# fergusfinn/qmps

Hardware: AMD Instinct MI355X
Metric: two-site energy evals/sec at D=4, batch=65536 (higher is better)
Workload: dtype f64

## Files before the change

### qmps_amd/csrc/qmps_direct.hip

```cpp
#include <hip/hip_runtime.h>
#include <stdint.h>

#include "qmps_hip.h"
#include "qmps_kernels.h"
#include "qmps_device.h"
#include "qmps_circuit.h"
#include "qmps_direct_core.h"
#include "qmps_direct_d8.h"

namespace qmps {

namespace {

struct QuadOps {
  using V = double;
  using P = bool;
  int q;
  const double2* row;
  double* gj;
  __device__ __forceinline__ P q_eq(int i) const { return q == i; }
  __device__ __forceinline__ P q_gt(int i) const { return q > i; }
  template <int L>
  static __device__ __forceinline__ V bcast(V v) { return quad_bcast<L>(v); }
  template <int L, int K>
  __device__ __forceinline__ void row_bcast(const V (&r)[16], V (&out)[16]) const {
#ifdef QMPS_GJ_LDS
    constexpr int K0 = K & ~1;
    __builtin_amdgcn_wave_barrier();
    if (q == L) {
#pragma unroll
      for (int j = K0; j < 16; j += 2) *(double2*)&gj[j] = make_double2(r[j], r[j + 1]);
    }
    __builtin_amdgcn_wave_barrier();
#pragma unroll
    for (int j = K0; j < 16; j += 2) {
      const double2 t = *(const double2*)&gj[j];
      if (j >= K) out[j] = t.x;
      out[j + 1] = t.y;
    }
#else
#pragma unroll
    for (int j = K; j < 16; ++j) out[j] = quad_bcast<L>(r[j]);
#endif
  }
  static __device__ __forceinline__ V qsum(V v) { return quad_sum(v); }
  static __device__ __forceinline__ V qmax(V v) {
    v = fmax(v, quad_perm<0xB1>(v));
    return fmax(v, quad_perm<0x4E>(v));
  }
  static __device__ __forceinline__ V vabs(V v) { return fabs(v); }
  static __device__ __forceinline__ V vmax(V a, V b) { return fmax(a, b); }
  static __device__ __forceinline__ V sel(P p, V a, V b) { return p ? a : b; }
  static __device__ __forceinline__ V splat(double x) { return x; }
  static __device__ __forceinline__ V fma(V a, V b, V c) { return dfma(a, b, c); }
  static __device__ __forceinline__ V rcp(V t) { return fast_rcp(t); }
  static __device__ __forceinline__ P lt(V a, V b) { return a < b; }
  static __device__ __forceinline__ P gt0(V a) { return a > 0.0; }
  static __device__ __forceinline__ P p_and(P a, P b) { return a && b; }
  static __device__ __forceinline__ P p_not(P a) { return !a; }
  static __device__ __forceinline__ bool any(P a) { return __any(a) != 0; }
  __device__ __forceinline__ void own(int s, int j, V& re, V& im) const {
    const double2 v = row[(4 * s + q) * 4 + j];
    re = v.x;
    im = v.y;
  }
  __device__ __forceinline__ void uni(int s, int i, int j, V& re, V& im) const {
    const double2 v = row[(4 * s + i) * 4 + j];
    re = v.x;
    im = v.y;
  }
};

typedef const __attribute__((address_space(4))) double* const_f64_ptr;
__device__ __forceinline__ const_f64_ptr h_term(const void* h, int t) { return (const_f64_ptr)(uintptr_t)h + 32 * t; }

typedef double v4f64 __attribute__((ext_vector_type(4)));
constexpr int kSqLD = 17;
constexpr int kSqDoubles = 16 * kSqLD + 16;

__device__ __forceinline__ void squaring_fallback(const unsigned char* tiles, int pad, double* img, int lane, bool todo,
                                                  int max_iter, double tol2, double (&x)[4], double& steps, bool& left) {
  constexpr int D = 4, LD = kSqLD;
  constexpr double RS2 = 0.70710678118654752, S2 = 1.4142135623730951;
  const int g = lane >> 4, c = lane & 15, j = c >> 2, jp = c & 3, q = lane & 3;
  double* strip = img + 16 * LD;
  const double cpx = j == jp ? 1.0 : (j < jp ? RS2 : 0.0), cpy = j > jp ? -RS2 : 0.0;
  const double cqx = j < jp ? RS2 : 0.0, cqy = j > jp ? RS2 : 0.0;
  const bool diag = j == jp;
  unsigned long long mask = __ballot(todo);
  while (mask != 0) {
    const int e = (__ffsll((long long)mask) - 1) >> 2;
    mask &= ~(0xFull << (4 * e));
    const double2* sA = (const double2*)(tiles + e * pad);
    v4f64 R;
    {
      double pr[2], pi[2], qr[2], qi[2];
#pragma unroll
      for (int s = 0; s < 2; ++s) {
        const double2 a = sA[(s * D + g) * D + jp], b = sA[(s * D + g) * D + j];
        pr[s] = dfma(cpx, a.x, cpy * a.y);
// ... 39 lines not shown
      ++m;
      image(acc);
      z = 0.25 * ((img[c * LD + 0] + img[c * LD + 5]) + (img[c * LD + 10] + img[c * LD + 15]));
      const double inv = fast_rcp(row16_sum(diag ? z : 0.0));
      z *= inv;
      R = acc * inv;
#pragma unroll
      for (int kk = 0; kk < 4; ++kk) af[kk] *= inv;
      const double d = z - prev;
      const double d2 = row16_sum(d * d);
      prev = z;
      st = (double)(1 << m);
      active = !(d2 < tol2);
    }
    __builtin_amdgcn_wave_barrier();
    if (lane < 16) strip[lane] = diag ? z : RS2 * z;
    __builtin_amdgcn_wave_barrier();
    if ((lane >> 2) == e) {
      if (m > 0) {
#pragma unroll
        for (int l = 0; l < 4; ++l) x[l] = strip[4 * q + l];
      }
      steps = 1.0 + st;
      left = active;
    }
  }
}

}

#ifndef QMPS_DIRECT_MINWAVES
#define QMPS_DIRECT_MINWAVES 2
#endif
template <int ANS, bool WARM>
__global__ __launch_bounds__(64, QMPS_DIRECT_MINWAVES) void energy_direct_d4_kernel(LaneArgs p) {
  using Core = DirectD4<QuadOps>;
  constexpr int ROW = 512, PAD = ROW + 16, ITEMS = 16;
  __shared__ __attribute__((aligned(16))) unsigned char lds[ITEMS * PAD];
  __shared__ double sq_img[kSqDoubles];
#ifdef QMPS_GJ_LDS
  __shared__ __attribute__((aligned(16))) double gjbuf[ITEMS * 18];
#endif
  const int lane = threadIdx.x, e = lane >> 2, q = lane & 3;
  const int64_t first = (int64_t)blockIdx.x * ITEMS;
  const int64_t b = first + e;
  const bool valid = b < p.B;
  if constexpr (ANS >= 0) {
    Reg<3> reg;
#pragma unroll
    for (int xx = 0; xx < 8; ++xx) {
      reg.re[xx] = (valid && xx == q) ? 1.0 : 0.0;
      reg.im[xx] = 0.0;
    }
    const int nsh = p.ans_nsh;
    const int64_t row = valid ? b : 0;
    const int64_t ridx = nsh > 0 ? row / nsh : row;
    const int shift_k = nsh > 0 ? (int)(row - ridx * nsh) : 0;
    const int isel = nsh > 0 ? *p.ans_i : -1;
    const double* pp = p.ans_params + ridx * p.ans_P;
    constexpr int per = ANS == QMPS_ANSATZ_SHALLOW_CNOT3 ? 3 : 2, trip = ANS == QMPS_ANSATZ_SHALLOW_CNOT3 ? 3 : 4;
    const int P = p.ans_P;
    for (int l = 0; l + per <= P; l += trip) {
      const int mine = l + q;
      double ang = 0.0;
      if (q < trip && mine < P) {
        ang = pp[mine];
        if (mine == isel) ang += roto_shift_value(nsh, shift_k);
      }
      const double scale = ansatz_angle_scale<ANS>(ANS == QMPS_ANSATZ_SHALLOW_CNOT3 ? q : (q & 1));
      double sn, cs;
      sincos(scale * ang, &sn, &cs);
      {
        const double c0[3] = {quad_bcast<0>(cs), quad_bcast<1>(cs), quad_bcast<2>(cs)};
        const double s0[3] = {quad_bcast<0>(sn), quad_bcast<1>(sn), quad_bcast<2>(sn)};
        ansatz_layer_cs<3, ANS>(reg, c0, s0);
      }
      if (trip == 4 && l + 2 + per <= P) {
        const double c1[2] = {quad_bcast<2>(cs), quad_bcast<3>(cs)};
        const double s1[2] = {quad_bcast<2>(sn), quad_bcast<3>(sn)};
        ansatz_layer_cs<3, ANS>(reg, c1, s1);
      }
    }
    double2* tile = (double2*)(lds + e * PAD);
#pragma unroll
    for (int xx = 0; xx < 8; ++xx) tile[((xx & 1) * 4 + (xx >> 1)) * 4 + q] = make_double2(reg.re[xx], reg.im[xx]);
  } else {
    const unsigned char* slab = (const unsigned char*)p.A + first * ROW;
    const int64_t slab_bytes = (p.B - first < ITEMS ? p.B - first : ITEMS) * (int64_t)ROW;
    double2 v[ITEMS * ROW / 1024];
#pragma unroll
    for (int c = 0; c < ITEMS * ROW / 1024; ++c) {
      const int off = c * 1024 + lane * 16;
      v[c] = make_double2(0.0, 0.0);
      if (off < slab_bytes) v[c] = *(const double2*)(slab + off);
    }
#pragma unroll
    for (int c = 0; c < ITEMS * ROW / 1024; ++c) {
      const int off = c * 1024 + lane * 16;
      *(double2*)(lds + (off / ROW) * PAD + (off % ROW)) = v[c];
    }
  }
  __syncthreads();
#ifdef QMPS_GJ_LDS
  const QuadOps o{q, (const double2*)(lds + e * PAD), gjbuf + e * 18};
#else
  const QuadOps o{q, (const double2*)(lds + e * PAD), nullptr};
#endif
  const double tol2 = p.tol * p.tol;

  double x[4], us[16];
  double steps = 1.0;
  int status = QMPS_ST_OK;
  bool have = false;
  if constexpr (WARM) {
    const double2* rin = (const double2*)p.r_in + (valid ? b : 0) * 16;
#pragma unroll
    for (int l = 0; l < 4; ++l) {
      const double2 rw = rin[q * 4 + l], cl = rin[l * 4 + q];
      x[l] = q <= l ? rw.x : cl.y;
    }
    Core::normalise(o, x);
    Core::gather(x, us);
    double y[4];
    const double d2 = Core::power_step(o, x, us, y);
    have = valid && d2 < tol2;
#pragma unroll
    for (int l = 0; l < 4; ++l) x[l] = have ? y[l] : x[l];
    __builtin_amdgcn_sched_barrier(0);
  }
  if (!WARM || __any(valid && !have)) {
    double Rc[4][16], xs[4], y[4];
    Core::build(o, Rc);
    __builtin_amdgcn_sched_barrier(0);
    double pivmax;
    Core::solve(o, Rc, xs, pivmax);
    __builtin_amdgcn_sched_barrier(0);
    Core::normalise(o, xs);
    Core::gather(xs, us);
    const double d2 = Core::power_step(o, xs, us, y);
    __builtin_amdgcn_sched_barrier(0);
    const bool accepted = d2 < tol2 && pivmax < Core::kMaxInversePivot;
    if (!have) {
#pragma unroll
      for (int l = 0; l < 4; ++l) x[l] = xs[l];
      if (WARM) steps = 2.0;
    }
    const bool todo = valid && !have && !accepted;
    if (__any(todo)) {
      bool left = false;
      squaring_fallback(lds, PAD, sq_img, lane, todo, p.max_iter - 1, tol2, x, steps, left);
      if (__any(todo && left)) {
        double yb[4];
        Core::gather(x, us);
        const double d2b = Core::power_step(o, x, us, yb);
        const bool fin = todo && left && d2b < tol2 && steps + 1.0 <= (double)p.max_iter;
#pragma unroll
        for (int l = 0; l < 4; ++l) x[l] = fin ? yb[l] : x[l];
        if (fin) {
          left = false;
          steps += 1.0;
        }
      }
      if (todo) {
        status = left ? QMPS_ST_NOT_CONVERGED : QMPS_ST_OK;
        if (WARM) steps += 1.0;
      }
    }
    if (WARM || __any(todo)) Core::gather(x, us);
  } else {
    Core::gather(x, us);
  }
  __builtin_amdgcn_sched_barrier(0);

  double pre[4][4], pim[4][4];
  const bool pd = Core::density(o, us, p.rho_need, pre, pim);
  if (status == QMPS_ST_OK && !pd) status = QMPS_ST_NOT_PD;
  if (p.acc_zero != nullptr && blockIdx.x == 0) acc_clear(p.acc_zero, p.n_terms, lane, 64);
  for (int t = 0; t < p.n_terms; ++t) {
    const double en = quad_sum(Core::energy(h_term(p.h, t), p.rho_need, pre, pim));
    if (valid && q == 0) p.E[b * p.n_terms + t] = en;
    if (p.partial != nullptr || p.acc != nullptr) {
      const double s = wave_sum((valid && q == 0) ? en : 0.0);
      if (lane == 0) {
        if (p.partial != nullptr) p.partial[(int64_t)t * gridDim.x + blockIdx.x] = s;
        if (p.acc != nullptr) acc_arrive(p.acc, p.acc_shards, t, blockIdx.x, s, p.acc_bound, p.acc_scale);
      }
    }
  }
  if (p.rho_out != nullptr) {
    double fre[4][4], fim[4][4];
#pragma unroll
    for (int t = 0; t < 4; ++t)
#pragma unroll
      for (int s = t; s < 4; ++s) {
        fre[t][s] = quad_sum(pre[t][s]);
        fim[t][s] = t == s ? 0.0 : quad_sum(pim[t][s]);
      }
    if (valid && q == 0) {
      double2* o2 = (double2*)p.rho_out + b * 16;
#pragma unroll
      for (int t = 0; t < 4; ++t)
#pragma unroll
        for (int s = 0; s < 4; ++s)
          o2[t * 4 + s] = t <= s ? make_double2(fre[t][s], fim[t][s]) : make_double2(fre[s][t], -fim[s][t]);
    }
  }
  if (!valid) return;
  if (q == 0) {
    p.iters[b] = (int32_t)steps;
    p.status[b] = status;
  }
  if (p.r_out != nullptr) {
    double2* o2 = (double2*)p.r_out + b * 16 + q * 4;
#pragma unroll
    for (int l = 0; l < 4; ++l) {
      const double f = q == 0 ? us[4 * l] : (q == 1 ? us[4 * l + 1] : (q == 2 ? us[4 * l + 2] : us[4 * l + 3]));
      const double re = q <= l ? x[l] : f;
      const double im = q == l ? 0.0 : (q < l ? f : -x[l]);
      o2[l] = make_double2(re, im);
    }
  }
// ... 349 lines not shown
```

### qmps_amd/csrc/qmps_direct_core.h

```cpp
#pragma once

#include <stdint.h>

#include <utility>

namespace qmps {

constexpr uint32_t kRhoNeedAll = 0xFFFFFFFFu;
inline uint32_t rho_need_mask(const double* h, int n_terms) {
  uint32_t need = 0;
  for (int n = 0; n < n_terms; ++n)
    for (int s = 0; s < 4; ++s)
      for (int t = 0; t < 4; ++t) {
        const int lo = t < s ? t : s, hi = t < s ? s : t;
        const double re = h[32 * n + 2 * (4 * s + t)], im = h[32 * n + 2 * (4 * s + t) + 1];
        if (!(re == 0.0)) need |= 1u << (4 * lo + hi);
        if (lo != hi && !(im == 0.0)) need |= 1u << (16 + 4 * lo + hi);
      }
  return need;
}

#if defined(__HIPCC__)
#define QMPS_CORE_FN __device__ inline __attribute__((always_inline))
#define QMPS_SCHED_FENCE() __builtin_amdgcn_sched_barrier(0)
#else
#define QMPS_CORE_FN inline __attribute__((always_inline))
#define QMPS_SCHED_FENCE() ((void)0)
#endif
#if defined(__HIP_DEVICE_COMPILE__)
#define QMPS_COMPUTED_HERE(v) asm volatile("" : "+v"(v))
#else
#define QMPS_COMPUTED_HERE(v) ((void)0)
#endif

template <int... I, class F>
QMPS_CORE_FN void static_for_impl(std::integer_sequence<int, I...>, F&& f) {
  (f(std::integral_constant<int, I>{}), ...);
}
template <int N, class F>
QMPS_CORE_FN void static_for(F&& f) {
  static_for_impl(std::make_integer_sequence<int, N>{}, static_cast<F&&>(f));
}

template <class O>
struct DirectD4 {
  using V = typename O::V;
  using P = typename O::P;

  static QMPS_CORE_FN V own_diag(const O& o, const V (&x)[4]) {
    return O::sel(o.q_eq(0), x[0], O::sel(o.q_eq(1), x[1], O::sel(o.q_eq(2), x[2], x[3])));
  }

  static QMPS_CORE_FN void build(const O& o, V (&Rc)[4][16]) {
    V ar[2][4], ai[2][4];
#pragma unroll
    for (int s = 0; s < 2; ++s)
#pragma unroll
      for (int j = 0; j < 4; ++j) o.own(s, j, ar[s][j], ai[s][j]);
#pragma unroll
    for (int ip = 0; ip < 4; ++ip) {
      const P rot = o.q_gt(ip);
      V tr[2][4], ti[2][4], br[2][4], bi[2][4];
#pragma unroll
      for (int s = 0; s < 2; ++s)
#pragma unroll
        for (int j = 0; j < 4; ++j) {
          tr[s][j] = ip == 3 ? ar[s][j] : O::sel(rot, -ai[s][j], ar[s][j]);
          ti[s][j] = ip == 3 ? ai[s][j] : O::sel(rot, ar[s][j], ai[s][j]);
          o.uni(s, ip, j, br[s][j], bi[s][j]);
        }
#pragma unroll
      for (int j = 0; j < 4; ++j) {
        V v = tr[0][j] * br[0][j];
        v = O::fma(ti[0][j], bi[0][j], v);
        v = O::fma(tr[1][j], br[1][j], v);
        v = O::fma(ti[1][j], bi[1][j], v);
        Rc[ip][5 * j] = v;
      }
#pragma unroll
      for (int lo = 0; lo < 4; ++lo)
// ... 5 lines not shown
            if (s > 0) {
              re = O::fma(tr[s][lo], br[s][hi], re);
              im = O::fma(tr[s][lo], bi[s][hi], im);
            }
            re = O::fma(ti[s][lo], bi[s][hi], re);
            re = O::fma(tr[s][hi], br[s][lo], re);
            re = O::fma(ti[s][hi], bi[s][lo], re);
            im = O::fma(-ti[s][lo], br[s][hi], im);
            im = O::fma(ti[s][hi], br[s][lo], im);
            im = O::fma(-tr[s][hi], bi[s][lo], im);
          }
          Rc[ip][4 * lo + hi] = re;
          Rc[ip][4 * hi + lo] = im;
        }
    }
  }

  static QMPS_CORE_FN void solve(const O& o, V (&M)[4][16], V (&x)[4], V& pivmax) {
    V y[4], dinv[4];
    const V one = O::splat(1.0), zero = O::splat(0.0);
    V w[4];
#pragma unroll
    for (int l = 0; l < 4; ++l) w[l] = O::sel(o.q_eq(l), one, zero);
#pragma unroll
    for (int r = 0; r < 4; ++r) {
#pragma unroll
      for (int l = 0; l < 4; ++l) M[r][4 * l + r] = M[r][4 * l + r] - w[l];
      dinv[r] = zero;
    }
#pragma unroll
    for (int j = 0; j < 4; ++j) M[3][5 * j] = M[3][5 * j] + w[3];
    static_for<16>([&](auto K) {
      constexpr int k = decltype(K)::value, pl = k >> 2, pr = k & 3;
      V prow[16];
      o.template row_bcast<pl, k>(M[pr], prow);
      const V pinv = O::rcp(prow[k]);
      const P mine = o.q_eq(pl);
      dinv[pr] = O::sel(mine, pinv, dinv[pr]);
#pragma unroll
      for (int r = 0; r < 4; ++r) {
        V f = M[r][k] * pinv;
        if (r == pr) f = O::sel(mine, zero, f);
#pragma unroll
        for (int j = k + 1; j < 16; ++j) M[r][j] = O::fma(-f, prow[j], M[r][j]);
        if (k == 15) y[r] = -f;
      }
    });
    y[3] = O::sel(o.q_eq(3), one, y[3]);
#pragma unroll
    for (int r = 0; r < 4; ++r) x[r] = y[r] * dinv[r];
    pivmax = O::qmax(O::vmax(O::vmax(O::vabs(dinv[0]), O::vabs(dinv[1])), O::vmax(O::vabs(dinv[2]), O::vabs(dinv[3]))));
  }

  static constexpr double kMaxInversePivot = 1e10;

  static QMPS_CORE_FN void gather(const V (&x)[4], V (&xs)[16]) {
    static_for<4>([&](auto L) {
      constexpr int l = decltype(L)::value;
#pragma unroll
      for (int r = 0; r < 4; ++r) xs[4 * l + r] = O::template bcast<l>(x[r]);
    });
  }

  static QMPS_CORE_FN V normalise(const O& o, V (&x)[4]) {
    const V tr = O::qsum(own_diag(o, x));
    const V inv = O::rcp(tr);
#pragma unroll
    for (int r = 0; r < 4; ++r) x[r] = x[r] * inv;
    return inv;
  }

  static QMPS_CORE_FN V dist2(const O& o, const V (&x)[4], const V (&y)[4]) {
    V d = O::splat(0.0);
#pragma unroll
    for (int r = 0; r < 4; ++r) {
      const V dd = y[r] - x[r];
      const V wt = O::sel(o.q_eq(r), O::splat(1.0), O::splat(2.0));
      d = O::fma(wt * dd, dd, d);
    }
    return O::qsum(d);
  }

  static QMPS_CORE_FN V power_step(const O& o, const V (&x)[4], const V (&us)[16], V (&y)[4]) {
    V ar[2][4], ai[2][4], xr[2][4], xi[2][4];
#pragma unroll
    for (int s = 0; s < 2; ++s)
#pragma unroll
      for (int j = 0; j < 4; ++j) o.own(s, j, ar[s][j], ai[s][j]);
#pragma unroll
    for (int s = 0; s < 2; ++s)
#pragma unroll
      for (int l = 0; l < 4; ++l) {
        V cr = O::splat(0.0), ci = O::splat(0.0);
#pragma unroll
        for (int k = 0; k < 4; ++k) {
          const V rr = us[k <= l ? 4 * k + l : 4 * l + k];
          cr = O::fma(ar[s][k], rr, cr);
          ci = O::fma(ai[s][k], rr, ci);
          if (k != l) {
            const V ri = k < l ? us[4 * l + k] : -us[4 * k + l];
            cr = O::fma(-ai[s][k], ri, cr);
            ci = O::fma(ar[s][k], ri, ci);
          }
        }
        xr[s][l] = cr;
        xi[s][l] = ci;
      }
#pragma unroll
    for (int l = 0; l < 4; ++l) {
      V cr = O::splat(0.0), ci = O::splat(0.0);
#pragma unroll
      for (int s = 0; s < 2; ++s)
#pragma unroll
        for (int k = 0; k < 4; ++k) {
          V br, bi;
          o.uni(s, l, k, br, bi);
          cr = O::fma(xr[s][k], br, cr);
          cr = O::fma(xi[s][k], bi, cr);
          ci = O::fma(xi[s][k], br, ci);
          ci = O::fma(-xr[s][k], bi, ci);
        }
      y[l] = l == 3 ? cr : O::sel(o.q_gt(l), -ci, cr);
    }
    normalise(o, y);
    return dist2(o, x, y);
  }

  static QMPS_CORE_FN void square(V (&Rc)[4][16]) {
    V out[4][16];
    static_for<16>([&](auto C) {
      constexpr int c = decltype(C)::value, cl = c >> 2, cr = c & 3;
      V rowc[16];
#pragma unroll
      for (int j = 0; j < 16; ++j) rowc[j] = O::template bcast<cl>(Rc[cr][j]);
#pragma unroll
      for (int r = 0; r < 4; ++r)
#pragma unroll
        for (int j = 0; j < 16; ++j) out[r][j] = c == 0 ? Rc[r][c] * rowc[j] : O::fma(Rc[r][c], rowc[j], out[r][j]);
      QMPS_SCHED_FENCE();
    });
#pragma unroll
    for (int r = 0; r < 4; ++r)
#pragma unroll
      for (int j = 0; j < 16; ++j) Rc[r][j] = out[r][j];
  }

  static QMPS_CORE_FN P squaring(const O& o, V (&Rc)[4][16], P active, int max_iter, double tol2, V (&x)[4], V& steps) {
    V prev[4];
#pragma unroll
    for (int r = 0; r < 4; ++r) prev[r] = O::sel(o.q_eq(r), O::splat(0.25), O::splat(0.0));
    int m = 0;
    while (O::any(active) && m < 29 && (2 << m) <= max_iter) {
      square(Rc);
      ++m;
      V z[4];
#pragma unroll
      for (int r = 0; r < 4; ++r) z[r] = O::splat(0.25) * ((Rc[r][0] + Rc[r][5]) + (Rc[r][10] + Rc[r][15]));
      const V inv = normalise(o, z);
#pragma unroll
      for (int r = 0; r < 4; ++r)
#pragma unroll
        for (int j = 0; j < 16; ++j) Rc[r][j] = Rc[r][j] * inv;
      const P conv = O::lt(dist2(o, prev, z), O::splat(tol2));
#pragma unroll
      for (int r = 0; r < 4; ++r) {
        x[r] = O::sel(active, z[r], x[r]);
        prev[r] = z[r];
      }
      steps = O::sel(active, O::splat((double)(1 << m)), steps);
      active = O::p_and(active, O::p_not(conv));
    }
    return active;
  }

  static QMPS_CORE_FN void b_rows(const O& o, V (&bre)[4][4], V (&bim)[4][4]) {
    V ar[2][4], ai[2][4];
#pragma unroll
    for (int s = 0; s < 2; ++s)
#pragma unroll
      for (int j = 0; j < 4; ++j) o.own(s, j, ar[s][j], ai[s][j]);
#pragma unroll
    for (int t2 = 0; t2 < 2; ++t2)
#pragma unroll
      for (int j = 0; j < 4; ++j) {
        V ur[4], ui[4];
#pragma unroll
        for (int k = 0; k < 4; ++k) o.uni(t2, j, k, ur[k], ui[k]);
#pragma unroll
        for (int t1 = 0; t1 < 2; ++t1)
#pragma unroll
          for (int k = 0; k < 4; ++k) {
            V cr, ci;
            if (j == 0) {
              cr = ar[t1][0] * ur[k];
              ci = ar[t1][0] * ui[k];
            } else {
              cr = O::fma(ar[t1][j], ur[k], bre[2 * t1 + t2][k]);
              ci = O::fma(ar[t1][j], ui[k], bim[2 * t1 + t2][k]);
            }
            bre[2 * t1 + t2][k] = O::fma(-ai[t1][j], ui[k], cr);
            bim[2 * t1 + t2][k] = O::fma(ai[t1][j], ur[k], ci);
          }
      }
  }

  static QMPS_CORE_FN V energy_lean(const V (&bre)[4][4], const V (&bim)[4][4], const V (&us)[16], const double* h) {
    V e = O::splat(0.0);
#pragma unroll
    for (int sg = 0; sg < 4; ++sg) {
      V cr[4], ci[4];
#pragma unroll
      for (int l = 0; l < 4; ++l) {
        cr[l] = O::splat(0.0);
        ci[l] = O::splat(0.0);
      }
#pragma unroll
      for (int tau = 0; tau < 4; ++tau) {
        const V hr = O::splat(h[2 * (4 * sg + tau)]), hi = O::splat(h[2 * (4 * sg + tau) + 1]);
#pragma unroll
        for (int l = 0; l < 4; ++l) {
          cr[l] = O::fma(hr, bre[tau][l], cr[l]);
          cr[l] = O::fma(-hi, bim[tau][l], cr[l]);
          ci[l] = O::fma(hr, bim[tau][l], ci[l]);
          ci[l] = O::fma(hi, bre[tau][l], ci[l]);
        }
      }
#pragma unroll
      for (int l = 0; l < 4; ++l) {
        V zr = O::splat(0.0), zi = O::splat(0.0);
#pragma unroll
        for (int k = 0; k < 4; ++k) {
          const V rr = us[k <= l ? 4 * k + l : 4 * l + k];
          zr = O::fma(cr[k], rr, zr);
          zi = O::fma(ci[k], rr, zi);
          if (k != l) {
            const V ri = k < l ? us[4 * l + k] : -us[4 * k + l];
            zr = O::fma(-ci[k], ri, zr);
            zi = O::fma(cr[k], ri, zi);
          }
        }
        e = O::fma(zr, bre[sg][l], e);
        e = O::fma(zi, bim[sg][l], e);
      }
    }
    return e;
  }

  static QMPS_CORE_FN P density(const O& o, const V (&us)[16], V (&pre)[4][4], V (&pim)[4][4]) {
    return density(o, us, kRhoNeedAll, pre, pim);
  }
  static QMPS_CORE_FN P density(const O& o, const V (&us)[16], uint32_t need, V (&pre)[4][4], V (&pim)[4][4]) {
    V rre[4][4], rim[4][4];
#pragma unroll
    for (int k = 0; k < 4; ++k)
#pragma unroll
      for (int l = k; l < 4; ++l) {
        rre[k][l] = us[4 * k + l];
        rim[k][l] = k == l ? O::splat(0.0) : us[4 * l + k];
      }
    P pd = O::gt0(rre[0][0]);
    V lre[4][4], lim[4][4], d[4];
    {
#pragma unroll
      for (int j = 0; j < 4; ++j) {
        V dj = rre[j][j];
#pragma unroll
        for (int k = 0; k < j; ++k) dj = O::fma(-(lre[j][k] * lre[j][k] + lim[j][k] * lim[j][k]), d[k], dj);
        d[j] = dj;
        pd = O::p_and(pd, O::gt0(dj));
        const V inv = O::rcp(O::sel(O::gt0(dj), dj, O::splat(1.0)));
#pragma unroll
        for (int i = j + 1; i < 4; ++i) {
          V cr = rre[j][i], ci = -rim[j][i];
#pragma unroll
          for (int k = 0; k < j; ++k) {
            const V pr = lre[i][k] * lre[j][k] + lim[i][k] * lim[j][k];
            const V pi = lim[i][k] * lre[j][k] - lre[i][k] * lim[j][k];
            cr = O::fma(-pr, d[k], cr);
            ci = O::fma(-pi, d[k], ci);
          }
          lre[i][j] = cr * inv;
          lim[i][j] = ci * inv;
        }
      }
    }
    V bre[4][4], bim[4][4];
    b_rows(o, bre, bim);
#pragma unroll
    for (int tau = 0; tau < 4; ++tau)
#pragma unroll
      for (int k = 0; k < 4; ++k) {
        V cr = bre[tau][k], ci = bim[tau][k];
#pragma unroll
        for (int i = k + 1; i < 4; ++i) {
          cr = O::fma(bre[tau][i], lre[i][k], cr);
          cr = O::fma(-bim[tau][i], lim[i][k], cr);
          ci = O::fma(bre[tau][i], lim[i][k], ci);
          ci = O::fma(bim[tau][i], lre[i][k], ci);
        }
        bre[tau][k] = cr;
        bim[tau][k] = ci;
      }
    computed_here(bre, bim);
#pragma unroll
    for (int tau = 0; tau < 4; ++tau) {
      V gre[4], gim[4];
#pragma unroll
      for (int k = 0; k < 4; ++k) {
        gre[k] = bre[tau][k] * d[k];
        gim[k] = bim[tau][k] * d[k];
      }
      rho_row(tau, need, gre, gim, bre, bim, pre, pim);
    }
    QMPS_SCHED_FENCE();
    if (O::any(O::p_not(pd))) {
      b_rows(o, bre, bim);
      computed_here(bre, bim);
#pragma unroll
      for (int tau = 0; tau < 4; ++tau) {
        V yre[4], yim[4];
#pragma unroll
        for (int l = 0; l < 4; ++l) {
          V cr = O::splat(0.0), ci = O::splat(0.0);
#pragma unroll
          for (int k = 0; k < 4; ++k) {
            const V rr = k <= l ? rre[k][l] : rre[l][k];
            cr = O::fma(bre[tau][k], rr, cr);
            ci = O::fma(bim[tau][k], rr, ci);
            if (k != l) {
              const V ri = k < l ? rim[k][l] : -rim[l][k];
              cr = O::fma(-bim[tau][k], ri, cr);
              ci = O::fma(bre[tau][k], ri, ci);
            }
          }
          yre[l] = cr;
          yim[l] = ci;
          QMPS_COMPUTED_HERE(yre[l]);
          QMPS_COMPUTED_HERE(yim[l]);
        }
        V qre[4][4], qim[4][4];
        rho_row(tau, need, yre, yim, bre, bim, qre, qim);
#pragma unroll
        for (int sg = tau; sg < 4; ++sg) {
          pre[tau][sg] = O::sel(pd, pre[tau][sg], qre[tau][sg]);
          pim[tau][sg] = O::sel(pd, pim[tau][sg], qim[tau][sg]);
        }
// ... 19 lines not shown
  }
  static QMPS_CORE_FN void rho_row(int tau, uint32_t need, const V (&yre)[4], const V (&yim)[4], const V (&bre)[4][4],
                                   const V (&bim)[4][4], V (&pre)[4][4], V (&pim)[4][4]) {
#pragma unroll
    for (int sg = tau; sg < 4; ++sg) {
      V cr = O::splat(0.0);
      if ((need >> (4 * tau + sg)) & 1u) {
        cr = yre[0] * bre[sg][0];
        cr = O::fma(yim[0], bim[sg][0], cr);
#pragma unroll
        for (int l = 1; l < 4; ++l) {
          cr = O::fma(yre[l], bre[sg][l], cr);
          cr = O::fma(yim[l], bim[sg][l], cr);
        }
      }
      pre[tau][sg] = cr;
      pim[tau][sg] = O::splat(0.0);
    }
    if ((need >> (16 + 4 * tau)) & 0xFu) {
#pragma unroll
      for (int sg = tau + 1; sg < 4; ++sg)
        if ((need >> (16 + 4 * tau + sg)) & 1u) {
          V ci = O::splat(0.0);
#pragma unroll
          for (int l = 0; l < 4; ++l) {
            ci = O::fma(yim[l], bre[sg][l], ci);
            ci = O::fma(-yre[l], bim[sg][l], ci);
          }
          pim[tau][sg] = ci;
        }
    }
  }

  static QMPS_CORE_FN V energy(const double* h, const V (&pre)[4][4], const V (&pim)[4][4]) {
    return energy(h, kRhoNeedAll, pre, pim);
  }
  template <class H>
  static QMPS_CORE_FN V energy(H h, uint32_t need, const V (&pre)[4][4], const V (&pim)[4][4]) {
    V e = O::splat(0.0);
    if ((need >> 16) != 0u) {
#pragma unroll
      for (int s = 0; s < 4; ++s) {
#pragma unroll
        for (int t = 0; t < 4; ++t) {
          const double hr = h[2 * (4 * s + t)], hi = h[2 * (4 * s + t) + 1];
          const V rr = t <= s ? pre[t][s] : pre[s][t];
          e = O::fma(O::splat(hr), rr, e);
          if (t != s) {
            const V ri = t < s ? pim[t][s] : -pim[s][t];
            e = O::fma(O::splat(-hi), ri, e);
          }
        }
        QMPS_COMPUTED_HERE(e);
      }
    } else {
#pragma unroll
      for (int s = 0; s < 4; ++s)
#pragma unroll
        for (int t = 0; t < 4; ++t) e = O::fma(O::splat(h[2 * (4 * s + t)]), t <= s ? pre[t][s] : pre[s][t], e);
    }
    return e;
  }
};

}
```

Before: 2.421 billion.

## Prefetch next row of unitary operands in power step and b_rows

Restructures power_step and b_rows so the LDS row reads for the next iteration are issued one step ahead into a double buffer, with sched_barrier hints marking where reads have been issued. The aim is to hide LDS latency behind the FMA work of the current row. It also splits the LDL factorisation out of density into helpers and adds optional phase-clock timing instrumentation that compiles out by default. The double buffering raises register pressure under a launch bound of 64 threads with two waves minimum, which could cause spills.

```diff
diff --git a/qmps_amd/csrc/qmps_direct.hip b/qmps_amd/csrc/qmps_direct.hip
--- a/qmps_amd/csrc/qmps_direct.hip
+++ b/qmps_amd/csrc/qmps_direct.hip
@@ -5,6 +5,35 @@
 #include "qmps_kernels.h"
 #include "qmps_device.h"
 #include "qmps_circuit.h"
+
+#ifdef QMPS_PHASE_CLOCK
+namespace qmps {
+constexpr int kPhaseStamps = 16;
+__device__ unsigned long long* g_phase_clock = nullptr;
+__device__ long long g_phase_clock_waves = 0;
+__shared__ unsigned long long phase_clock_lds[kPhaseStamps];
+__device__ __forceinline__ void phase_stamp(int i) {
+  __builtin_amdgcn_sched_barrier(0);
+  unsigned long long t;
+  asm volatile("s_memtime %0\n\ts_waitcnt lgkmcnt(0)" : "=s"(t)::"memory");
+  if (threadIdx.x == 0) phase_clock_lds[i] = t;
+  __builtin_amdgcn_sched_barrier(0);
+}
+__device__ __forceinline__ void phase_flush() {
+  unsigned long long* buf = g_phase_clock;
+  __builtin_amdgcn_wave_barrier();
+  if (buf != nullptr && threadIdx.x < kPhaseStamps && (long long)blockIdx.x < g_phase_clock_waves)
+    buf[(size_t)blockIdx.x * kPhaseStamps + threadIdx.x] = phase_clock_lds[threadIdx.x];
+}
+}
+extern "C" int qmps_phase_clock_buffer(void* device_buffer, long long n_waves) {
+  if (device_buffer == nullptr) n_waves = 0;
+  hipError_t e = hipMemcpyToSymbol(HIP_SYMBOL(qmps::g_phase_clock_waves), &n_waves, sizeof(n_waves));
+  if (e == hipSuccess) e = hipMemcpyToSymbol(HIP_SYMBOL(qmps::g_phase_clock), &device_buffer, sizeof(device_buffer));
+  return (int)e;
+}
+#define QMPS_PHASE_CLOCK_STAMP(i) ::qmps::phase_stamp(i)
+#endif
 #include "qmps_direct_core.h"
 #include "qmps_direct_d8.h"
 
@@ -171,9 +200,12 @@
 #ifndef QMPS_DIRECT_MINWAVES
 #define QMPS_DIRECT_MINWAVES 2
 #endif
+#ifndef QMPS_DIRECT_AHEAD
+#define QMPS_DIRECT_AHEAD (kAheadPower | kAheadRows)
+#endif
 template <int ANS, bool WARM>
 __global__ __launch_bounds__(64, QMPS_DIRECT_MINWAVES) void energy_direct_d4_kernel(LaneArgs p) {
-  using Core = DirectD4<QuadOps>;
+  using Core = DirectD4<QuadOps, QMPS_DIRECT_AHEAD>;
   constexpr int ROW = 512, PAD = ROW + 16, ITEMS = 16;
   __shared__ __attribute__((aligned(16))) unsigned char lds[ITEMS * PAD];
   __shared__ double sq_img[kSqDoubles];
@@ -184,6 +216,7 @@
   const int64_t first = (int64_t)blockIdx.x * ITEMS;
   const int64_t b = first + e;
   const bool valid = b < p.B;
+  QMPS_PHASE_STAMP(0);
   if constexpr (ANS >= 0) {
     Reg<3> reg;
 #pragma unroll
@@ -240,6 +273,7 @@
     }
   }
   __syncthreads();
+  QMPS_PHASE_STAMP(1);
 #ifdef QMPS_GJ_LDS
   const QuadOps o{q, (const double2*)(lds + e * PAD), gjbuf + e * 18};
 #else
@@ -270,13 +304,17 @@
   if (!WARM || __any(valid && !have)) {
     double Rc[4][16], xs[4], y[4];
     Core::build(o, Rc);
+    QMPS_PHASE_STAMP(2, phase_pin(Rc));
     __builtin_amdgcn_sched_barrier(0);
     double pivmax;
     Core::solve(o, Rc, xs, pivmax);
+    QMPS_PHASE_STAMP(6, phase_pin(xs), phase_pin(pivmax));
     __builtin_amdgcn_sched_barrier(0);
     Core::normalise(o, xs);
     Core::gather(xs, us);
+    QMPS_PHASE_STAMP(7, phase_pin(us));
     const double d2 = Core::power_step(o, xs, us, y);
+    QMPS_PHASE_STAMP(9, phase_pin(y));
     __builtin_amdgcn_sched_barrier(0);
     const bool accepted = d2 < tol2 && pivmax < Core::kMaxInversePivot;
     if (!have) {
@@ -326,6 +364,10 @@
       }
     }
   }
+  QMPS_PHASE_STAMP(15);
+#ifdef QMPS_PHASE_CLOCK
+  phase_flush();
+#endif
   if (p.rho_out != nullptr) {
     double fre[4][4], fim[4][4];
 #pragma unroll
diff --git a/qmps_amd/csrc/qmps_direct_core.h b/qmps_amd/csrc/qmps_direct_core.h
--- a/qmps_amd/csrc/qmps_direct_core.h
+++ b/qmps_amd/csrc/qmps_direct_core.h
@@ -27,12 +27,50 @@
 #define QMPS_CORE_FN inline __attribute__((always_inline))
 #define QMPS_SCHED_FENCE() ((void)0)
 #endif
+#if defined(__HIPCC__)
+#define QMPS_READS_ISSUED() __builtin_amdgcn_sched_barrier(4)
+#else
+#define QMPS_READS_ISSUED() ((void)0)
+#endif
 #if defined(__HIP_DEVICE_COMPILE__)
 #define QMPS_COMPUTED_HERE(v) asm volatile("" : "+v"(v))
 #else
 #define QMPS_COMPUTED_HERE(v) ((void)0)
 #endif
 
+#ifdef QMPS_PHASE_CLOCK_STAMP
+#define QMPS_PHASE_STAMP(i, ...) \
+  do {                           \
+    __VA_ARGS__;                 \
+    QMPS_PHASE_CLOCK_STAMP(i);   \
+  } while (0)
+template <class T>
+QMPS_CORE_FN void phase_pin(T& v) {
+  QMPS_COMPUTED_HERE(v);
+}
+template <int FROM = 0, class T, int N>
+QMPS_CORE_FN void phase_pin(T (&a)[N]) {
+#pragma unroll
+  for (int i = FROM; i < N; ++i) QMPS_COMPUTED_HERE(a[i]);
+}
+template <int FROM = 0, bool LOWER = false, class T, int N, int M>
+QMPS_CORE_FN void phase_pin(T (&a)[N][M]) {
+#pragma unroll
+  for (int i = 0; i < N; ++i)
+#pragma unroll
+    for (int j = FROM; j < (LOWER ? i : M); ++j) QMPS_COMPUTED_HERE(a[i][j]);
+}
+template <class T, int N>
+QMPS_CORE_FN void phase_pin_upper(T (&a)[N][N]) {
+#pragma unroll
+  for (int i = 0; i < N; ++i)
+#pragma unroll
+    for (int j = i; j < N; ++j) QMPS_COMPUTED_HERE(a[i][j]);
+}
+#else
+#define QMPS_PHASE_STAMP(...) ((void)0)
+#endif
+
 template <int... I, class F>
 QMPS_CORE_FN void static_for_impl(std::integer_sequence<int, I...>, F&& f) {
   (f(std::integral_constant<int, I>{}), ...);
@@ -42,10 +80,16 @@
   static_for_impl(std::make_integer_sequence<int, N>{}, static_cast<F&&>(f));
 }
 
-template <class O>
+constexpr int kAheadPower = 1, kAheadRows = 2;
+template <class O, int AHEAD = 0>
 struct DirectD4 {
   using V = typename O::V;
   using P = typename O::P;
+
+  template <int WHICH>
+  static QMPS_CORE_FN void reads_issued() {
+    if constexpr ((AHEAD & WHICH) != 0) QMPS_READS_ISSUED();
+  }
 
   static QMPS_CORE_FN V own_diag(const O& o, const V (&x)[4]) {
     return O::sel(o.q_eq(0), x[0], O::sel(o.q_eq(1), x[1], O::sel(o.q_eq(2), x[2], x[3])));
@@ -117,6 +161,7 @@
     for (int j = 0; j < 4; ++j) M[3][5 * j] = M[3][5 * j] + w[3];
     static_for<16>([&](auto K) {
       constexpr int k = decltype(K)::value, pl = k >> 2, pr = k & 3;
+      if constexpr (k >= 4 && pr == 0) QMPS_PHASE_STAMP(2 + pl, phase_pin<k>(M), phase_pin(dinv));
       V prow[16];
       o.template row_bcast<pl, k>(M[pr], prow);
       const V pinv = O::rcp(prow[k]);
@@ -168,47 +213,71 @@
 
   static QMPS_CORE_FN V power_step(const O& o, const V (&x)[4], const V (&us)[16], V (&y)[4]) {
     V ar[2][4], ai[2][4], xr[2][4], xi[2][4];
+    constexpr bool ahead = (AHEAD & kAheadPower) != 0;
+    V br[2][2][4], bi[2][2][4];
+    power_own(o, ar, ai);
+    if (ahead) power_rows(o, 0, br[0], bi[0]);
+    reads_issued<kAheadPower>();
+#pragma unroll
+    for (int s = 0; s < 2; ++s) power_left(s, ar, ai, us, xr, xi);
+    reads_issued<kAheadPower>();
+#pragma unroll
+    for (int l = 0; l < 4; ++l) {
+      const int c = ahead ? l & 1 : 0;
+      if (!ahead) power_rows(o, l, br[c], bi[c]);
+      else if (l < 3) power_rows(o, l + 1, br[c ^ 1], bi[c ^ 1]);
+      reads_issued<kAheadPower>();
+      power_right(o, l, xr, xi, br[c], bi[c], y);
+      reads_issued<kAheadPower>();
+    }
+    QMPS_PHASE_STAMP(8, phase_pin(y));
+    normalise(o, y);
+    return dist2(o, x, y);
+  }
+  static QMPS_CORE_FN void power_own(const O& o, V (&ar)[2][4], V (&ai)[2][4]) {
 #pragma unroll
     for (int s = 0; s < 2; ++s)
 #pragma unroll
       for (int j = 0; j < 4; ++j) o.own(s, j, ar[s][j], ai[s][j]);
-#pragma unroll
-    for (int s = 0; s < 2; ++s)
-#pragma unroll
-      for (int l = 0; l < 4; ++l) {
-        V cr = O::splat(0.0), ci = O::splat(0.0);
-#pragma unroll
-        for (int k = 0; k < 4; ++k) {
-          const V rr = us[k <= l ? 4 * k + l : 4 * l + k];
-          cr = O::fma(ar[s][k], rr, cr);
-          ci = O::fma(ai[s][k], rr, ci);
-          if (k != l) {
-            const V ri = k < l ? us[4 * l + k] : -us[4 * k + l];
-            cr = O::fma(-ai[s][k], ri, cr);
-            ci = O::fma(ar[s][k], ri, ci);
-          }
-        }
-        xr[s][l] = cr;
-        xi[s][l] = ci;
-      }
+  }
+  static QMPS_CORE_FN void power_left(int s, const V (&ar)[2][4], const V (&ai)[2][4], const V (&us)[16], V (&xr)[2][4], V (&xi)[2][4]) {
 #pragma unroll
     for (int l = 0; l < 4; ++l) {
       V cr = O::splat(0.0), ci = O::splat(0.0);
 #pragma unroll
-      for (int s = 0; s < 2; ++s)
-#pragma unroll
-        for (int k = 0; k < 4; ++k) {
-          V br, bi;
-          o.uni(s, l, k, br, bi);
-          cr = O::fma(xr[s][k], br, cr);
-          cr = O::fma(xi[s][k], bi, cr);
-          ci = O::fma(xi[s][k], br, ci);
-          ci = O::fma(-xr[s][k], bi, ci);
-        }
-      y[l] = l == 3 ? cr : O::sel(o.q_gt(l), -ci, cr);
-    }
-    normalise(o, y);
-    return dist2(o, x, y);
+      for (int k = 0; k < 4; ++k) {
+        const V rr = us[k <= l ? 4 * k + l : 4 * l + k];
+        cr = O::fma(ar[s][k], rr, cr);
+        ci = O::fma(ai[s][k], rr, ci);
+        if (k != l) {
+          const V ri = k < l ? us[4 * l + k] : -us[4 * k + l];
+          cr = O::fma(-ai[s][k], ri, cr);
+          ci = O::fma(ar[s][k], ri, ci);
+        }
+      }
+      xr[s][l] = cr;
+      xi[s][l] = ci;
+    }
+  }
+  static QMPS_CORE_FN void power_rows(const O& o, int l, V (&br)[2][4], V (&bi)[2][4]) {
+#pragma unroll
+    for (int s = 0; s < 2; ++s)
+#pragma unroll
+      for (int k = 0; k < 4; ++k) o.uni(s, l, k, br[s][k], bi[s][k]);
+  }
+  static QMPS_CORE_FN void power_right(const O& o, int l, const V (&xr)[2][4], const V (&xi)[2][4], const V (&br)[2][4], const V (&bi)[2][4],
+                                       V (&y)[4]) {
+    V cr = O::splat(0.0), ci = O::splat(0.0);
+#pragma unroll
+    for (int s = 0; s < 2; ++s)
+#pragma unroll
+      for (int k = 0; k < 4; ++k) {
+        cr = O::fma(xr[s][k], br[s][k], cr);
+        cr = O::fma(xi[s][k], bi[s][k], cr);
+        ci = O::fma(xi[s][k], br[s][k], ci);
+        ci = O::fma(-xr[s][k], bi[s][k], ci);
+      }
+    y[l] = l == 3 ? cr : O::sel(o.q_gt(l), -ci, cr);
   }
 
   static QMPS_CORE_FN void square(V (&Rc)[4][16]) {
@@ -264,29 +333,38 @@
     for (int s = 0; s < 2; ++s)
 #pragma unroll
       for (int j = 0; j < 4; ++j) o.own(s, j, ar[s][j], ai[s][j]);
-#pragma unroll
-    for (int t2 = 0; t2 < 2; ++t2)
-#pragma unroll
-      for (int j = 0; j < 4; ++j) {
-        V ur[4], ui[4];
-#pragma unroll
-        for (int k = 0; k < 4; ++k) o.uni(t2, j, k, ur[k], ui[k]);
-#pragma unroll
-        for (int t1 = 0; t1 < 2; ++t1)
-#pragma unroll
-          for (int k = 0; k < 4; ++k) {
-            V cr, ci;
-            if (j == 0) {
-              cr = ar[t1][0] * ur[k];
-              ci = ar[t1][0] * ui[k];
-            } else {
-              cr = O::fma(ar[t1][j], ur[k], bre[2 * t1 + t2][k]);
-              ci = O::fma(ar[t1][j], ui[k], bim[2 * t1 + t2][k]);
-            }
-            bre[2 * t1 + t2][k] = O::fma(-ai[t1][j], ui[k], cr);
-            bim[2 * t1 + t2][k] = O::fma(ai[t1][j], ur[k], ci);
+    constexpr bool ahead = (AHEAD & kAheadRows) != 0;
+    V ur[2][4], ui[2][4];
+    if (ahead) {
+#pragma unroll
+      for (int k = 0; k < 4; ++k) o.uni(0, 0, k, ur[0][k], ui[0][k]);
+    }
+#pragma unroll
+    for (int p = 0; p < 8; ++p) {
+      const int t2 = p >> 2, j = p & 3, c = ahead ? p & 1 : 0;
+      const int pn = ahead ? p + 1 : p, n = ahead ? c ^ 1 : 0;
+      if (pn < 8) {
+#pragma unroll
+        for (int k = 0; k < 4; ++k) o.uni(pn >> 2, pn & 3, k, ur[n][k], ui[n][k]);
+      }
+      reads_issued<kAheadRows>();
+#pragma unroll
+      for (int t1 = 0; t1 < 2; ++t1)
+#pragma unroll
+        for (int k = 0; k < 4; ++k) {
+          V cr, ci;
+          if (j == 0) {
+            cr = ar[t1][0] * ur[c][k];
+            ci = ar[t1][0] * ui[c][k];
+          } else {
+            cr = O::fma(ar[t1][j], ur[c][k], bre[2 * t1 + t2][k]);
+            ci = O::fma(ar[t1][j], ui[c][k], bim[2 * t1 + t2][k]);
           }
-      }
+          bre[2 * t1 + t2][k] = O::fma(-ai[t1][j], ui[c][k], cr);
+          bim[2 * t1 + t2][k] = O::fma(ai[t1][j], ur[c][k], ci);
+        }
+      reads_issued<kAheadRows>();
+    }
   }
 
   static QMPS_CORE_FN V energy_lean(const V (&bre)[4][4], const V (&bim)[4][4], const V (&us)[16], const double* h) {
@@ -335,6 +413,50 @@
     return density(o, us, kRhoNeedAll, pre, pim);
   }
   static QMPS_CORE_FN P density(const O& o, const V (&us)[16], uint32_t need, V (&pre)[4][4], V (&pim)[4][4]) {
+    QMPS_PHASE_STAMP(10);
+    V lre[4][4], lim[4][4], d[4];
+    const P pd = ldl(us, lre, lim, d);
+    QMPS_PHASE_STAMP(11, (phase_pin<0, true>(lre)), (phase_pin<0, true>(lim)), phase_pin(d));
+    return density_from(o, us, lre, lim, d, pd, need, pre, pim);
+  }
+
+  static QMPS_CORE_FN P ldl(const V (&us)[16], V (&lre)[4][4], V (&lim)[4][4], V (&d)[4]) {
+    P pd = O::gt0(us[0]);
+#pragma unroll
+    for (int j = 0; j < 4; ++j) ldl_column(j, us, lre, lim, d, pd);
+    return pd;
+  }
+  static QMPS_CORE_FN V ab_plus(V a, V b, V c) {
+#if defined(__HIP_DEVICE_COMPILE__)
+    return O::fma(a, b, c);
+#else
+    return a * b + c;
+#endif
+  }
+  static QMPS_CORE_FN void ldl_column(int j, const V (&us)[16], V (&lre)[4][4], V (&lim)[4][4], V (&d)[4], P& pd) {
+    V dj = us[5 * j];
+#pragma unroll
+    for (int k = 0; k < j; ++k) dj = O::fma(-ab_plus(lre[j][k], lre[j][k], lim[j][k] * lim[j][k]), d[k], dj);
+    d[j] = dj;
+    pd = O::p_and(pd, O::gt0(dj));
+    const V inv = O::rcp(O::sel(O::gt0(dj), dj, O::splat(1.0)));
+#pragma unroll
+    for (int i = j + 1; i < 4; ++i) {
+      V cr = us[4 * j + i], ci = -us[4 * i + j];
+#pragma unroll
+      for (int k = 0; k < j; ++k) {
+        const V pr = ab_plus(lre[i][k], lre[j][k], lim[i][k] * lim[j][k]);
+        const V pi = ab_plus(lim[i][k], lre[j][k], -(lre[i][k] * lim[j][k]));
+        cr = O::fma(-pr, d[k], cr);
+        ci = O::fma(-pi, d[k], ci);
+      }
+      lre[i][j] = cr * inv;
+      lim[i][j] = ci * inv;
+    }
+  }
+
+  static QMPS_CORE_FN P density_from(const O& o, const V (&us)[16], const V (&lre)[4][4], const V (&lim)[4][4], const V (&d)[4], P pd,
+                                     uint32_t need, V (&pre)[4][4], V (&pim)[4][4]) {
     V rre[4][4], rim[4][4];
 #pragma unroll
     for (int k = 0; k < 4; ++k)
@@ -343,34 +465,9 @@
         rre[k][l] = us[4 * k + l];
         rim[k][l] = k == l ? O::splat(0.0) : us[4 * l + k];
       }
-    P pd = O::gt0(rre[0][0]);
-    V lre[4][4], lim[4][4], d[4];
-    {
-#pragma unroll
-      for (int j = 0; j < 4; ++j) {
-        V dj = rre[j][j];
-#pragma unroll
-        for (int k = 0; k < j; ++k) dj = O::fma(-(lre[j][k] * lre[j][k] + lim[j][k] * lim[j][k]), d[k], dj);
-        d[j] = dj;
-        pd = O::p_and(pd, O::gt0(dj));
-        const V inv = O::rcp(O::sel(O::gt0(dj), dj, O::splat(1.0)));
-#pragma unroll
-        for (int i = j + 1; i < 4; ++i) {
-          V cr = rre[j][i], ci = -rim[j][i];
-#pragma unroll
-          for (int k = 0; k < j; ++k) {
-            const V pr = lre[i][k] * lre[j][k] + lim[i][k] * lim[j][k];
-            const V pi = lim[i][k] * lre[j][k] - lre[i][k] * lim[j][k];
-            cr = O::fma(-pr, d[k], cr);
-            ci = O::fma(-pi, d[k], ci);
-          }
-          lre[i][j] = cr * inv;
-          lim[i][j] = ci * inv;
-        }
-      }
-    }
     V bre[4][4], bim[4][4];
     b_rows(o, bre, bim);
+    QMPS_PHASE_STAMP(12, computed_here(bre, bim));
 #pragma unroll
     for (int tau = 0; tau < 4; ++tau)
 #pragma unroll
@@ -387,6 +484,7 @@
         bim[tau][k] = ci;
       }
     computed_here(bre, bim);
+    QMPS_PHASE_STAMP(13);
 #pragma unroll
     for (int tau = 0; tau < 4; ++tau) {
       V gre[4], gim[4];
@@ -397,6 +495,7 @@
       }
       rho_row(tau, need, gre, gim, bre, bim, pre, pim);
     }
+    QMPS_PHASE_STAMP(14, phase_pin_upper(pre), phase_pin_upper(pim));
     QMPS_SCHED_FENCE();
     if (O::any(O::p_not(pd))) {
       b_rows(o, bre, bim);
```

Result: no change. 2.445 billion, median of 4 (+1.0%).

## Reuse power-step site products to build two-site density in cold path

Applied to the files above, without the earlier changes.

For the non-warm path, the power step now computes per-site partial products (SiteW) and keeps them, then builds the two-site reduced density from those factors plus column products of the unitary, instead of the full LDL-plus-b_rows density contraction. Only factors required by the Hamiltonian's need mask are computed, and the factors are refreshed after the squaring fallback for lanes that took it. The aim is to cut redundant FLOPs between the power step and the density evaluation. In exchange it keeps more registers live across the solve (SiteW holds 32 doubles), which may lower occupancy. The LDL factorisation is still run for the positive-definiteness check.

```diff
diff --git a/qmps_amd/csrc/qmps_direct.hip b/qmps_amd/csrc/qmps_direct.hip
--- a/qmps_amd/csrc/qmps_direct.hip
+++ b/qmps_amd/csrc/qmps_direct.hip
@@ -66,6 +66,11 @@
   }
   __device__ __forceinline__ void uni(int s, int i, int j, V& re, V& im) const {
     const double2 v = row[(4 * s + i) * 4 + j];
+    re = v.x;
+    im = v.y;
+  }
+  __device__ __forceinline__ void col(int s, int i, V& re, V& im) const {
+    const double2 v = row[(4 * s + i) * 4 + q];
     re = v.x;
     im = v.y;
   }
@@ -250,6 +255,7 @@
   double x[4], us[16];
   double steps = 1.0;
   int status = QMPS_ST_OK;
+  [[maybe_unused]] Core::SiteW W;
   bool have = false;
   if constexpr (WARM) {
     const double2* rin = (const double2*)p.r_in + (valid ? b : 0) * 16;
@@ -276,7 +282,9 @@
     __builtin_amdgcn_sched_barrier(0);
     Core::normalise(o, xs);
     Core::gather(xs, us);
-    const double d2 = Core::power_step(o, xs, us, y);
+    double d2;
+    if constexpr (WARM) d2 = Core::power_step(o, xs, us, y);
+    else d2 = Core::power_step_sites(o, xs, us, p.rho_need, y, W);
     __builtin_amdgcn_sched_barrier(0);
     const bool accepted = d2 < tol2 && pivmax < Core::kMaxInversePivot;
     if (!have) {
@@ -304,15 +312,21 @@
         status = left ? QMPS_ST_NOT_CONVERGED : QMPS_ST_OK;
         if (WARM) steps += 1.0;
       }
-    }
-    if (WARM || __any(todo)) Core::gather(x, us);
+      if constexpr (!WARM) {
+        Core::gather(x, us);
+        Core::update_sites(o, us, p.rho_need, todo, W);
+      }
+    }
+    if constexpr (WARM) Core::gather(x, us);
   } else {
     Core::gather(x, us);
   }
   __builtin_amdgcn_sched_barrier(0);
 
   double pre[4][4], pim[4][4];
-  const bool pd = Core::density(o, us, p.rho_need, pre, pim);
+  bool pd;
+  if constexpr (WARM) pd = Core::density(o, us, p.rho_need, pre, pim);
+  else pd = Core::density_sites(o, us, p.rho_need, W, pre, pim);
   if (status == QMPS_ST_OK && !pd) status = QMPS_ST_NOT_PD;
   if (p.acc_zero != nullptr && blockIdx.x == 0) acc_clear(p.acc_zero, p.n_terms, lane, 64);
   for (int t = 0; t < p.n_terms; ++t) {
diff --git a/qmps_amd/csrc/qmps_direct_core.h b/qmps_amd/csrc/qmps_direct_core.h
--- a/qmps_amd/csrc/qmps_direct_core.h
+++ b/qmps_amd/csrc/qmps_direct_core.h
@@ -18,6 +18,24 @@
         if (lo != hi && !(im == 0.0)) need |= 1u << (16 + 4 * lo + hi);
       }
   return need;
+}
+
+constexpr uint32_t kSiteN00 = 1u, kSiteN10 = 2u, kSiteN11 = 4u, kSiteW01 = 8u, kSiteW10 = 16u;
+constexpr uint32_t rho_site_parts(uint32_t factor) {
+  uint32_t parts = 0;
+  for (int tau = 0; tau < 4; ++tau)
+    for (int sg = tau; sg < 4; ++sg) {
+      const int t1 = tau >> 1, t2 = tau & 1, s1 = sg >> 1, s2 = sg & 1;
+      const uint32_t n = s1 == 0 ? kSiteN00 : (t1 == 0 ? kSiteN10 : kSiteN11);
+      const uint32_t w = t2 == s2 ? 0u : (t2 == 0 ? kSiteW01 : kSiteW10);
+      if (factor == n || factor == w) parts |= (1u << (4 * tau + sg)) | (sg != tau ? 1u << (16 + 4 * tau + sg) : 0u);
+    }
+  return parts;
+}
+constexpr uint32_t rho_site_factors(uint32_t need) {
+  return ((need & rho_site_parts(kSiteN00)) != 0u ? kSiteN00 : 0u) | ((need & rho_site_parts(kSiteN10)) != 0u ? kSiteN10 : 0u) |
+         ((need & rho_site_parts(kSiteN11)) != 0u ? kSiteN11 : 0u) | ((need & rho_site_parts(kSiteW01)) != 0u ? kSiteW01 : 0u) |
+         ((need & rho_site_parts(kSiteW10)) != 0u ? kSiteW10 : 0u);
 }
 
 #if defined(__HIPCC__)
@@ -167,7 +185,29 @@
   }
 
   static QMPS_CORE_FN V power_step(const O& o, const V (&x)[4], const V (&us)[16], V (&y)[4]) {
-    V ar[2][4], ai[2][4], xr[2][4], xi[2][4];
+    V xr[2][4], xi[2][4];
+    own_rows_times_r(o, us, xr, xi);
+#pragma unroll
+    for (int l = 0; l < 4; ++l) {
+      V cr = O::splat(0.0), ci = O::splat(0.0);
+#pragma unroll
+      for (int s = 0; s < 2; ++s)
+#pragma unroll
+        for (int k = 0; k < 4; ++k) {
+          V br, bi;
+          o.uni(s, l, k, br, bi);
+          cr = O::fma(xr[s][k], br, cr);
+          cr = O::fma(xi[s][k], bi, cr);
+          ci = O::fma(xi[s][k], br, ci);
+          ci = O::fma(-xr[s][k], bi, ci);
+        }
+      y[l] = l == 3 ? cr : O::sel(o.q_gt(l), -ci, cr);
+    }
+    normalise(o, y);
+    return dist2(o, x, y);
+  }
+  static QMPS_CORE_FN void own_rows_times_r(const O& o, const V (&us)[16], V (&xr)[2][4], V (&xi)[2][4]) {
+    V ar[2][4], ai[2][4];
 #pragma unroll
     for (int s = 0; s < 2; ++s)
 #pragma unroll
@@ -191,24 +231,62 @@
         xr[s][l] = cr;
         xi[s][l] = ci;
       }
+  }
+
+  struct SiteW {
+    V re[2][2][4], im[2][2][4];
+  };
+  static QMPS_CORE_FN V power_step_sites(const O& o, const V (&x)[4], const V (&us)[16], uint32_t need, V (&y)[4], SiteW& w) {
+    V xr[2][4], xi[2][4];
+    own_rows_times_r(o, us, xr, xi);
+    site_w(o, xr[0], xi[0], 0, w.re[0][0], w.im[0][0]);
+    site_w(o, xr[1], xi[1], 1, w.re[1][1], w.im[1][1]);
 #pragma unroll
     for (int l = 0; l < 4; ++l) {
-      V cr = O::splat(0.0), ci = O::splat(0.0);
-#pragma unroll
-      for (int s = 0; s < 2; ++s)
-#pragma unroll
-        for (int k = 0; k < 4; ++k) {
-          V br, bi;
-          o.uni(s, l, k, br, bi);
-          cr = O::fma(xr[s][k], br, cr);
-          cr = O::fma(xi[s][k], bi, cr);
-          ci = O::fma(xi[s][k], br, ci);
-          ci = O::fma(-xr[s][k], bi, ci);
-        }
-      y[l] = l == 3 ? cr : O::sel(o.q_gt(l), -ci, cr);
-    }
+      const V cr = w.re[0][0][l] + w.re[1][1][l];
+      y[l] = l == 3 ? cr : O::sel(o.q_gt(l), -(w.im[0][0][l] + w.im[1][1][l]), cr);
+    }
+    const uint32_t f = rho_site_factors(need);
+    if (f & kSiteW01) site_w(o, xr[0], xi[0], 1, w.re[0][1], w.im[0][1]);
+    if (f & kSiteW10) site_w(o, xr[1], xi[1], 0, w.re[1][0], w.im[1][0]);
     normalise(o, y);
     return dist2(o, x, y);
+  }
+  static QMPS_CORE_FN void site_w(const O& o, const V (&xr)[4], const V (&xi)[4], int s2, V (&wre)[4], V (&wim)[4]) {
+#pragma unroll
+    for (int l = 0; l < 4; ++l) {
+      V br, bi;
+      o.uni(s2, l, 0, br, bi);
+      V cr = O::fma(xi[0], bi, xr[0] * br), ci = O::fma(-xr[0], bi, xi[0] * br);
+#pragma unroll
+      for (int k = 1; k < 4; ++k) {
+        o.uni(s2, l, k, br, bi);
+        cr = O::fma(xr[k], br, cr);
+        cr = O::fma(xi[k], bi, cr);
+        ci = O::fma(xi[k], br, ci);
+        ci = O::fma(-xr[k], bi, ci);
+      }
+      wre[l] = cr;
+      wim[l] = ci;
+    }
+  }
+  static QMPS_CORE_FN void update_sites(const O& o, const V (&us)[16], uint32_t need, P p, SiteW& w) {
+    V xr[2][4], xi[2][4];
+    own_rows_times_r(o, us, xr, xi);
+    const uint32_t f = rho_site_factors(need);
+#pragma unroll
+    for (int t2 = 0; t2 < 2; ++t2)
+#pragma unroll
+      for (int s2 = 0; s2 < 2; ++s2) {
+        if (t2 != s2 && !(f & (t2 == 0 ? kSiteW01 : kSiteW10))) continue;
+        V tre[4], tim[4];
+        site_w(o, xr[t2], xi[t2], s2, tre, tim);
+#pragma unroll
+        for (int l = 0; l < 4; ++l) {
+          w.re[t2][s2][l] = O::sel(p, tre[l], w.re[t2][s2][l]);
+          w.im[t2][s2][l] = O::sel(p, tim[l], w.im[t2][s2][l]);
+        }
+      }
   }
 
   static QMPS_CORE_FN void square(V (&Rc)[4][16]) {
@@ -331,11 +409,7 @@
     return e;
   }
 
-  static QMPS_CORE_FN P density(const O& o, const V (&us)[16], V (&pre)[4][4], V (&pim)[4][4]) {
-    return density(o, us, kRhoNeedAll, pre, pim);
-  }
-  static QMPS_CORE_FN P density(const O& o, const V (&us)[16], uint32_t need, V (&pre)[4][4], V (&pim)[4][4]) {
-    V rre[4][4], rim[4][4];
+  static QMPS_CORE_FN P ldl(const V (&us)[16], V (&rre)[4][4], V (&rim)[4][4], V (&lre)[4][4], V (&lim)[4][4], V (&d)[4]) {
 #pragma unroll
     for (int k = 0; k < 4; ++k)
 #pragma unroll
@@ -344,31 +418,37 @@
         rim[k][l] = k == l ? O::splat(0.0) : us[4 * l + k];
       }
     P pd = O::gt0(rre[0][0]);
-    V lre[4][4], lim[4][4], d[4];
-    {
-#pragma unroll
-      for (int j = 0; j < 4; ++j) {
-        V dj = rre[j][j];
-#pragma unroll
-        for (int k = 0; k < j; ++k) dj = O::fma(-(lre[j][k] * lre[j][k] + lim[j][k] * lim[j][k]), d[k], dj);
-        d[j] = dj;
-        pd = O::p_and(pd, O::gt0(dj));
-        const V inv = O::rcp(O::sel(O::gt0(dj), dj, O::splat(1.0)));
-#pragma unroll
-        for (int i = j + 1; i < 4; ++i) {
-          V cr = rre[j][i], ci = -rim[j][i];
-#pragma unroll
-          for (int k = 0; k < j; ++k) {
-            const V pr = lre[i][k] * lre[j][k] + lim[i][k] * lim[j][k];
-            const V pi = lim[i][k] * lre[j][k] - lre[i][k] * lim[j][k];
-            cr = O::fma(-pr, d[k], cr);
-            ci = O::fma(-pi, d[k], ci);
-          }
-          lre[i][j] = cr * inv;
-          lim[i][j] = ci * inv;
-        }
-      }
-    }
+#pragma unroll
+    for (int j = 0; j < 4; ++j) {
+      V dj = rre[j][j];
+#pragma unroll
+      for (int k = 0; k < j; ++k) dj = O::fma(-(lre[j][k] * lre[j][k] + lim[j][k] * lim[j][k]), d[k], dj);
+      d[j] = dj;
+      pd = O::p_and(pd, O::gt0(dj));
+      const V inv = O::rcp(O::sel(O::gt0(dj), dj, O::splat(1.0)));
+#pragma unroll
+      for (int i = j + 1; i < 4; ++i) {
+        V cr = rre[j][i], ci = -rim[j][i];
+#pragma unroll
+        for (int k = 0; k < j; ++k) {
+          const V pr = lre[i][k] * lre[j][k] + lim[i][k] * lim[j][k];
+          const V pi = lim[i][k] * lre[j][k] - lre[i][k] * lim[j][k];
+          cr = O::fma(-pr, d[k], cr);
+          ci = O::fma(-pi, d[k], ci);
+        }
+        lre[i][j] = cr * inv;
+        lim[i][j] = ci * inv;
+      }
+    }
+    return pd;
+  }
+
+  static QMPS_CORE_FN P density(const O& o, const V (&us)[16], V (&pre)[4][4], V (&pim)[4][4]) {
+    return density(o, us, kRhoNeedAll, pre, pim);
+  }
+  static QMPS_CORE_FN P density(const O& o, const V (&us)[16], uint32_t need, V (&pre)[4][4], V (&pim)[4][4]) {
+    V rre[4][4], rim[4][4], lre[4][4], lim[4][4], d[4];
+    const P pd = ldl(us, rre, rim, lre, lim, d);
     V bre[4][4], bim[4][4];
     b_rows(o, bre, bim);
 #pragma unroll
@@ -482,6 +562,89 @@
     }
   }
 
+  static QMPS_CORE_FN P density_sites(const O& o, const V (&us)[16], uint32_t need, const SiteW& w, V (&pre)[4][4], V (&pim)[4][4]) {
+    P pd;
+    {
+      V rre[4][4], rim[4][4], lre[4][4], lim[4][4], d[4];
+      pd = ldl(us, rre, rim, lre, lim, d);
+    }
+#pragma unroll
+    for (int tau = 0; tau < 4; ++tau)
+#pragma unroll
+      for (int sg = tau; sg < 4; ++sg) {
+        pre[tau][sg] = O::splat(0.0);
+        pim[tau][sg] = O::splat(0.0);
+      }
+    static_for<3>([&](auto F) {
+      constexpr int s1 = decltype(F)::value == 0 ? 0 : 1, t1 = decltype(F)::value == 2 ? 1 : 0;
+      constexpr uint32_t parts = rho_site_parts(1u << decltype(F)::value);
+      if (need & parts) {
+        V cr[4], ci[4], nre[4], nim[4];
+#pragma unroll
+        for (int i = 0; i < 4; ++i) o.col(t1, i, cr[i], ci[i]);
+#pragma unroll
+        for (int l = 0; l < 4; ++l) {
+          V ur, ui;
+          o.uni(s1, 0, l, ur, ui);
+          V re = O::fma(ui, ci[0], ur * cr[0]), im = O::fma(-ui, cr[0], ur * ci[0]);
+#pragma unroll
+          for (int i = 1; i < 4; ++i) {
+            o.uni(s1, i, l, ur, ui);
+            re = O::fma(ur, cr[i], re);
+            re = O::fma(ui, ci[i], re);
+            im = O::fma(ur, ci[i], im);
+            im = O::fma(-ui, cr[i], im);
+          }
+          nre[l] = re;
+          nim[l] = im;
+        }
+#pragma unroll
+        for (int l = 0; l < 4; ++l) {
+          QMPS_COMPUTED_HERE(nre[l]);
+          QMPS_COMPUTED_HERE(nim[l]);
+        }
+#pragma unroll
+        for (int t2 = 0; t2 < 2; ++t2)
+#pragma unroll
+          for (int s2 = 0; s2 < 2; ++s2) {
+            const int tau = 2 * t1 + t2, sg = 2 * s1 + s2;
+            if (tau > sg) continue;
+            if ((need >> (4 * tau + sg)) & 1u) {
+              V c = w.re[t2][s2][0] * nre[0];
+              c = O::fma(-w.im[t2][s2][0], nim[0], c);
+#pragma unroll
+              for (int l = 1; l < 4; ++l) {
+                c = O::fma(w.re[t2][s2][l], nre[l], c);
+                c = O::fma(-w.im[t2][s2][l], nim[l], c);
+              }
+              pre[tau][sg] = c;
+            }
+          }
+        if ((need & parts) >> 16) {
+#pragma unroll
+          for (int t2 = 0; t2 < 2; ++t2)
+#pragma unroll
+            for (int s2 = 0; s2 < 2; ++s2) {
+              const int tau = 2 * t1 + t2, sg = 2 * s1 + s2;
+              if (tau >= sg) continue;
+              if ((need >> (16 + 4 * tau + sg)) & 1u) {
+                V c = w.re[t2][s2][0] * nim[0];
+                c = O::fma(w.im[t2][s2][0], nre[0], c);
+#pragma unroll
+                for (int l = 1; l < 4; ++l) {
+                  c = O::fma(w.re[t2][s2][l], nim[l], c);
+                  c = O::fma(w.im[t2][s2][l], nre[l], c);
+                }
+                pim[tau][sg] = c;
+              }
+            }
+        }
+      }
+    });
+    QMPS_SCHED_FENCE();
+    return pd;
+  }
+
   static QMPS_CORE_FN V energy(const double* h, const V (&pre)[4][4], const V (&pim)[4][4]) {
     return energy(h, kRhoNeedAll, pre, pim);
   }
```

New measurement: 2.449 billion before, 2.521 billion after (median of 6 runs). 2.9% higher.
